# jiahansu/GPUAR

Hardware: AMD Instinct MI355X
Metric: encode+decode GB/s (higher is better)
Workload: dtype u16

## Files before the change

gpuar_amd/csrc/gpuar_kernels.hip:

```cpp
#include <hip/hip_runtime.h>
#include <mutex>
#include <stdint.h>
#include <stdio.h>
#include <stdlib.h>
#include <string.h>

#include "gpuar_hip.h"

#include "lane_codec.h"
#include "crc32.h"
#include "planes.h"

namespace gpuar {

__constant__ RecipTable g_recip = RecipTable();
struct MulTable {
    uint32_t m[kPacket + 64];
    constexpr MulTable() : m{} {
        const RecipTable r = RecipTable();
        for (uint32_t i = 0; i < kPacket + 64; ++i) m[i] = r.r[i < kPacket ? i : kPacket - 1u].mul;
    }
};
__device__ const MulTable g_mul = MulTable();
__constant__ DecodeConstTable g_decode = DecodeConstTable();
__device__ uint32_t g_status = 0;
__device__ uint32_t g_status_taken;
__device__ uint32_t g_cu_ticket[2048];
constexpr uint32_t kClockSlots = 256, kClockEvery = 64;
__device__ unsigned long long g_clock_samples[2][kClockSlots][4];
__device__ __forceinline__ void clock_sample(uint32_t which, size_t group, uint32_t lane, uint32_t end) {
    if ((group & (kClockEvery - 1u)) == 0u && group < size_t(kClockSlots) * kClockEvery && lane == 0u) {
        unsigned long long *slot = g_clock_samples[which][group / kClockEvery] + 2u * end;
        slot[0] = clock64();
        slot[1] = wall_clock64();
    }
}

__device__ __forceinline__ uint32_t lane_column(uint32_t lane) {
    return ((lane & 31u) << 1) | (lane >> 5);
}

__device__ __forceinline__ uint32_t wave_max(uint32_t v) {
#pragma unroll
    for (int off = 32; off > 0; off >>= 1) {
        const uint32_t other = __shfl_xor(v, off);
        v = other > v ? other : v;
    }
    return __builtin_amdgcn_readfirstlane(v);
}

constexpr uint32_t kPhase = 8;
constexpr int kPrioTop = 3, kPrioCoder = 0, kPrioLow = 2;

constexpr uint32_t kRingSlots = 3;
struct alignas(16) EncodeLds {
    uint8_t tree[kTreeRows * kLanes * 2];
    uint32_t sums[kRingSlots][kPhase][kLanes];
    uint32_t bytes[2][kPhase / 4][kLanes];
};
__device__ __forceinline__ uint32_t next_slot(uint32_t slot) { return slot == kRingSlots - 1u ? 0u : slot + 1u; }

__device__ __forceinline__ size_t xcd_contiguous_group(uint32_t block, uint32_t grid) {
    const uint32_t per_xcd = grid >> 3;
    return static_cast<size_t>(block & 7u) * per_xcd + (block >> 3);
}

__device__ __forceinline__ void lds_barrier() {
    asm volatile("s_waitcnt lgkmcnt(0)\n\ts_barrier" ::: "memory");
}

__device__ __forceinline__ uint4 load16_guarded(const uint8_t *p, size_t avail) {
    if (avail >= 16) return *reinterpret_cast<const uint4 *>(p);
    uint32_t w[4] = {0, 0, 0, 0};
    for (size_t b = 0; b < avail; ++b) w[b >> 2] |= static_cast<uint32_t>(p[b]) << (8u * (b & 3u));
    return make_uint4(w[0], w[1], w[2], w[3]);
}
// ... 991 lines not shown

#define GPUAR_STREAM_EVEN_TAKE  \
            "v_add_u32 %[pc], %[no], %[ne]\n\t"  \
            "v_sub_co_u32 %[raw], %[sb], %[rem], %[pc]\n\t"  \
            "v_and_b32 %[rem], 31, %[raw]\n\t"
#define GPUAR_STREAM_EVEN_WINDOW  \
            "v_perm_b32 %[pa], 0, %[ahead], %[bsw]\n\t"  \
            "v_cndmask_b32 %[w0], %[w0], %[w1], %[sb]\n\t" \
            "v_cndmask_b32 %[w1], %[w1], %[pa], %[sb]\n\t" \
            "v_alignbit_b32 v216, %[w0], %[w1], %[rem]\n\t"
#define GPUAR_STREAM_ODD_MOVE  \
            "v_lshrrev_b32 %[pb], 31, %[raw]\n\t"  \
            "v_lshl_add_u32 %[next], %[pb], 8, %[next]\n\t" \
            "v_and_or_b32 %[pc], %[next], %[kf00], %[ring]\n\t"  \
            "ds_read_b32 %[ahead], %[pc]\n\t"

#define GPUAR_OFF_TEXT(N) \
            "v_lshlrev_b64 v[216:217], %[" N "], v[216:217]\n\t"

#define GPUAR_STEP_OPERANDS_COMMON \
              [R0] "=&v"(R0), [R] "=&v"(R), [np] "=&v"(np), [am] "=&v"(am), [t0] "=&v"(t0), [t1] "=&v"(t1), [t2] "=&v"(t2), [t3] "=&v"(t3), \
              [m0] "=&s"(m0), [m1] "=&s"(m1), [ma] "=&s"(ma), [mc] "=&s"(mc), [mj] "=&s"(mj), [sx] "=&s"(sx), [sb] "=&s"(sb), [raw] "+v"(rem_raw), \
              [root] "+v"(dec.model.root), [h0] "+v"(dec.model.half0), [h1] "+v"(dec.model.half1), \
              [rng] "+v"(dec.range), [off] "+v"(offr), [kff] "+v"(kff), [oaddr] "+v"(oaddr), \
              [rem] "+v"(dec.rem), [w0] "+v"(dec.w0), [w1] "+v"(dec.w1), [ahead] "+v"(dec.ahead), [next] "+v"(next64), "+v"(window), \
              [dn] "=&v"(dn), [bw] "=&v"(bw), [cc] "=&v"(cc), [pa] "=&v"(pa), [pb] "=&v"(pb), [pc] "=&v"(pc), [ps] "=&v"(ps), \
              [wd] "=&v"(wd), [h] "=&v"(h), [e] "=&v"(e)

#define GPUAR_STEP_LOCALS \
        uint32_t R0, R, np, am, t0, t1, t2, t3, dn, bw, cc, pa, pb, pc, ps, wd, h, e; \
        unsigned long long m0, m1, ma, mc, mj, sx, sb;

#define GPUAR_STEP_EVEN_TEXT(SHADOW, OWN_ADDRESS, J, MUL, WORD) \
    GPUAR_STEP_HEAD                                 \
    SHADOW GPUAR_TOTAL_STEP GPUAR_REG_NODES GPUAR_STREAM_EVEN_TAKE \
    "s_waitcnt lgkmcnt(1)\n\t"                      \
    GPUAR_MID_WALK                                  \
    GPUAR_STREAM_EVEN_WINDOW \
    "s_waitcnt lgkmcnt(1)\n\t"                      \
    GPUAR_LOW_WALK(OWN_ADDRESS) GPUAR_LOW_INTERVAL(MUL) GPUAR_STEP_END("ne") GPUAR_FILE_SYMBOL(J, WORD) GPUAR_OFF_TEXT("ne")
#define GPUAR_STEP_ODD_TEXT(SHADOW, OWN_ADDRESS, J, MUL, WORD) \
    GPUAR_STEP_HEAD \
    SHADOW GPUAR_TOTAL_STEP GPUAR_STREAM_ODD_MOVE \
    "s_waitcnt lgkmcnt(2)\n\t"                      \
    GPUAR_MID_WALK \
    GPUAR_REG_NODES \
    "s_waitcnt lgkmcnt(1)\n\t"                      \
    GPUAR_LOW_WALK(OWN_ADDRESS) GPUAR_LOW_INTERVAL(MUL) GPUAR_STEP_END("no") GPUAR_FILE_SYMBOL(J, WORD) GPUAR_OFF_TEXT("no")
#define GPUAR_STEP_FIRST(J, MUL, WORD) GPUAR_STEP_EVEN_TEXT(GPUAR_SHADOW_PLAIN, , J, MUL, WORD)
#define GPUAR_STEP_EVEN(J, MUL, WORD) GPUAR_STEP_EVEN_TEXT(GPUAR_SHADOW_DEFERRED, , J, MUL, WORD)
#define GPUAR_STEP_ODD(J, MUL, WORD) GPUAR_STEP_ODD_TEXT(GPUAR_SHADOW_DEFERRED, , J, MUL, WORD)
#define GPUAR_STEP_LAST(J, MUL, WORD) GPUAR_STEP_ODD_TEXT(GPUAR_SHADOW_DEFERRED, GPUAR_LOW_ADDRESS_NOW, J, MUL, WORD)

constexpr uint32_t kRingPieces = 4;
constexpr uint32_t kDecodeLdsQuads = (kDecodeRecords + kRingPieces) * kLanes;

template <bool kBatch = false>
__device__ __forceinline__ void decode_wave(uint8_t *col, uint8_t *ring, const uint8_t *base, uint32_t pkt_off, uint32_t limit_off,
                                            uint8_t *out, bool live, uint32_t *status, uint32_t room = kPacket) {
    DecoderLane<9> dec;
    dec.template open<kBatch>(col, base, pkt_off, limit_off, live, room);
    const uint32_t len_max = wave_max(dec.ulen);
    uint32_t i = 0;

    const uint32_t col_lds = static_cast<uint32_t>(reinterpret_cast<uintptr_t>(col));
    const uint32_t ring_lds = static_cast<uint32_t>(reinterpret_cast<uintptr_t>(ring));
    if ((ring_lds & 0xF00u) != 0u) {
        atomicOr(status, GPUAR_STATUS_BAD_PACKET);
        return;
    }
    register uint32_t o0 asm("v204");
    register uint32_t o1 asm("v205");
    register uint32_t offr asm("v217");
    offr = dec.off | (dec.lo << 16);
    uint32_t n_even = 0, n_odd = dec.owed_bits;
    uint32_t total_v = 256u;
    uint32_t rem_raw = 0;
    register uint32_t window asm("v216");
    asm volatile("v_mov_b32 %0, 0" : "=v"(window));
    const uint32_t col_low_lds = col_lds + SubtreeModel<9>::kLowBase;
    uint32_t oaddr = col_lds + dec.model.owed.at;
    uint32_t kff = 0xFFFFu;
    const uint32_t k64k = 0x10000u, k64k1 = 0x10001u;
    const uint32_t minus_half = 0xFFFF8000u;
    uint32_t bswap_sel, ring_wrap, low_half;
    asm volatile("s_mov_b32 %0, 0xffff" : "=s"(low_half));
    asm volatile("s_mov_b32 %0, 0x00010203" : "=s"(bswap_sel));
    asm volatile("s_movk_i32 %0, 0xf00" : "=s"(ring_wrap));

    const uint32_t skew16 = static_cast<uint32_t>(reinterpret_cast<uintptr_t>(base) & 15u);
    const uint8_t *base16 = base - skew16;
    const uint32_t next16 = dec.next + skew16;
    uint32_t next64 = (next16 - 4u) << 6;
    const uint32_t last_piece = (dec.last + skew16) & ~15u;
    const uint32_t first_piece = (next16 - 4u) & ~15u;
    uint32_t fill = first_piece + 16u * kRingPieces;
    register uint32_t q0 asm("v220");
    register uint32_t q1 asm("v221");
    register uint32_t q2 asm("v222");
    register uint32_t q3 asm("v223");
    uint32_t slot_lds = ring_lds;
#pragma unroll
    for (uint32_t k = 0; k < kRingPieces; ++k) {
        const uint32_t at = first_piece + 16u * k;
        const Quad q = load128(base16 + (at < last_piece ? at : last_piece));
        uint32_t *slot = reinterpret_cast<uint32_t *>(ring + ((at & 0x30u) << 6));
        slot[0] = q.w[0], slot[64] = q.w[1], slot[128] = q.w[2], slot[192] = q.w[3];
        if (k == kRingPieces - 1u) {
            q0 = q.w[0], q1 = q.w[1], q2 = q.w[2], q3 = q.w[3];
            slot_lds = ring_lds + ((at & 0x30u) << 6);
        }
    }
#define GPUAR_RING_PHASE_TEXT(TUPLE_LO, TUPLE_HI)                                                                    \
            "v_lshrrev_b32 %[rt], 6, %[next]\n\t"                                                                    \
            "v_sub_u32 %[rt], %[fill], %[rt]\n\t"                                                                    \
            "v_cmp_gt_u32 vcc, 49, %[rt]\n\t"  \
            "s_waitcnt vmcnt(0)\n\t"                                                                                 \
            "ds_write2st64_b32 %[slot], v220, v221 offset1:1\n\t"                                                    \
            "ds_write2st64_b32 %[slot], v222, v223 offset0:2 offset1:3\n\t"                                          \
            "global_load_dwordx4 " TUPLE_LO ", %[zero], %[mulbase] offset:%[roff]\n\t"                               \
            "global_load_dwordx4 " TUPLE_HI ", %[zero], %[mulbase] offset:%[roff]+16\n\t"                            \
            "s_and_saveexec_b64 %[sx], vcc\n\t"                                                                      \
            "v_min_u32 %[rt], %[fill], %[lastp]\n\t"                                                                 \
            "global_load_dwordx4 v[220:223], %[rt], %[base]\n\t"                                                     \
            "v_and_b32 %[t2], 48, %[fill]\n\t"                                                                       \
            "v_lshl_add_u32 %[slot], %[t2], 6, %[ring]\n\t"                                                          \
            "v_add_u32 %[fill], 16, %[fill]\n\t"                                                                     \
            "s_or_b64 exec, exec, %[sx]"

    register uint32_t m00 asm("v224"); register uint32_t m01 asm("v225"); register uint32_t m02 asm("v226"); register uint32_t m03 asm("v227"); register uint32_t m04 asm("v228"); register uint32_t m05 asm("v229"); register uint32_t m06 asm("v230"); register uint32_t m07 asm("v231");
    register uint32_t m10 asm("v232"); register uint32_t m11 asm("v233"); register uint32_t m12 asm("v234"); register uint32_t m13 asm("v235"); register uint32_t m14 asm("v236"); register uint32_t m15 asm("v237"); register uint32_t m16 asm("v238"); register uint32_t m17 asm("v239");
    register uint32_t m20 asm("v240"); register uint32_t m21 asm("v241"); register uint32_t m22 asm("v242"); register uint32_t m23 asm("v243"); register uint32_t m24 asm("v244"); register uint32_t m25 asm("v245"); register uint32_t m26 asm("v246"); register uint32_t m27 asm("v247");
    register uint32_t m30 asm("v248"); register uint32_t m31 asm("v249"); register uint32_t m32 asm("v250"); register uint32_t m33 asm("v251"); register uint32_t m34 asm("v252"); register uint32_t m35 asm("v253"); register uint32_t m36 asm("v254"); register uint32_t m37 asm("v255");
    uint32_t vzero;
    asm volatile("v_mov_b32 %0, 0" : "=v"(vzero));
#define GPUAR_DECODE_RUN8(RUN, FIRST_KIND, LAST_KIND, WORD_A, WORD_B, SET_AHEAD, TUPLE_LO, TUPLE_HI)                         \
        {                                                                                                            \
            GPUAR_STEP_LOCALS                                                                                        \
            uint32_t lbw_, lcc_, ti_, path7_, rt_;                                                                   \
            unsigned long long lma_;                                                                                 \
            asm volatile(                                                                                            \
                FIRST_KIND(0, "mul0", "wa") GPUAR_STEP_ODD(1, "mul1", "wa") GPUAR_STEP_EVEN(2, "mul2", "wa") GPUAR_STEP_ODD(3, "mul3", "wa") \
                GPUAR_STEP_EVEN(0, "mul4", "wb") GPUAR_STEP_ODD(1, "mul5", "wb") GPUAR_STEP_EVEN(2, "mul6", "wb") LAST_KIND(3, "mul7", "wb") \
                 \
                GPUAR_RING_PHASE_TEXT(TUPLE_LO, TUPLE_HI)                                                            \
                : GPUAR_STEP_OPERANDS_COMMON,                                                                        \
                  [lbw] "=&v"(lbw_), [lcc] "=&v"(lcc_), [ti] "=&v"(ti_), [lma] "=&s"(lma_), [wa] "+v"(WORD_A), [wb] "+v"(WORD_B),     \
                  "+v"(o0), "+v"(o1), [c6] "+v"(path6), [c7] "=&v"(path7_), [ne] "+v"(n_even), [no] "+v"(n_odd), [totv] "+v"(total_v), \
                  [slot] "+v"(slot_lds), [fill] "+v"(fill), [rt] "=&v"(rt_), "+v"(q0), "+v"(q1), "+v"(q2), "+v"(q3),               \
                  "=v"(m##SET_AHEAD##0), "=v"(m##SET_AHEAD##1), "=v"(m##SET_AHEAD##2), "=v"(m##SET_AHEAD##3),                     \
                  "=v"(m##SET_AHEAD##4), "=v"(m##SET_AHEAD##5), "=v"(m##SET_AHEAD##6), "=v"(m##SET_AHEAD##7)                      \
                : [mul0] "v"(m##RUN##0), [mul1] "v"(m##RUN##1), [mul2] "v"(m##RUN##2), [mul3] "v"(m##RUN##3),                     \
                  [mul4] "v"(m##RUN##4), [mul5] "v"(m##RUN##5), [mul6] "v"(m##RUN##6), [mul7] "v"(m##RUN##7),                     \
                  [shift] "s"(block_shift), [col] "v"(col_lds), [collow] "v"(col_low_lds), [ring] "v"(ring_lds),                  \
                  [k64k] "v"(k64k), [k64k1] "v"(k64k1), [bsw] "s"(bswap_sel), [kf00] "s"(ring_wrap), [km32k] "s"(minus_half), [kffff] "s"(low_half), \
                  [lastp] "v"(last_piece), [base] "s"(base16), [zero] "v"(vzero), [mulbase] "s"(mul_base), [roff] "n"(32 * ((RUN) + 2))   \
                : "vcc", "scc", "memory", "v200", "v201", "v202", "v203", "v208", "v209", "v212", "v213", "v214", "v215");         \
        }
#define GPUAR_DECODE_BLOCK                                                                                           \
    {                                                                                                                \
         \
        const uint32_t block_shift = 30u - static_cast<uint32_t>(__builtin_clz(256u + i));                           \
        total_v = 256u + i;               \
        asm volatile("" : "+v"(total_v));                                                                            \
        _Pragma("unroll 1") for (uint32_t half = 0; half < 2u; ++half) {                                             \
            const uint32_t *mul_base = g_mul.m + i + 32u * half;                   \
             \
             \
            uint32_t path6;                                                                                          \
            asm volatile("" : "=v"(path6));                                                                          \
            GPUAR_DECODE_RUN8(0, GPUAR_STEP_FIRST, GPUAR_STEP_ODD, w0, w1, 2, "v[240:243]", "v[244:247]")            \
            GPUAR_DECODE_RUN8(1, GPUAR_STEP_EVEN, GPUAR_STEP_ODD, w2, w3, 3, "v[248:251]", "v[252:255]")             \
            GPUAR_DECODE_RUN8(2, GPUAR_STEP_EVEN, GPUAR_STEP_ODD, w4, w5, 0, "v[224:227]", "v[228:231]")             \
            GPUAR_DECODE_RUN8(3, GPUAR_STEP_EVEN, GPUAR_STEP_LAST, w6, w7, 1, "v[232:235]", "v[236:239]")            \
             \
             \
             \
            if (half == 0u) {                                                                                        \
                k0 = ~w0, k1 = ~w1, k2 = ~w2, k3 = ~w3, k4 = ~w4, k5 = ~w5, k6 = ~w6, k7 = ~w7;                      \
            } else {                                                                                                 \
                uint4 *dst = reinterpret_cast<uint4 *>(out + i);                                                     \
                dst[0] = make_uint4(k0, k1, k2, k3);                                                                 \
                dst[1] = make_uint4(k4, k5, k6, k7);                                                                 \
                dst[2] = make_uint4(~w0, ~w1, ~w2, ~w3);                                                             \
                dst[3] = make_uint4(~w4, ~w5, ~w6, ~w7);                                                             \
            }                                                                                                        \
        }                                                                                                            \
    }

    const uint32_t len_min = wave_max(~dec.ulen) ^ 0xFFFFFFFFu;
    asm volatile("v_mov_b32 %0, 0\n\tv_mov_b32 %1, 0" : "=v"(o0), "=v"(o1));
    uint32_t w0, w1, w2, w3, w4, w5, w6, w7;
    uint32_t k0 = 0, k1 = 0, k2 = 0, k3 = 0, k4 = 0, k5 = 0, k6 = 0, k7 = 0;
    asm volatile("v_mov_b32 %0, 0\n\tv_mov_b32 %1, 0\n\tv_mov_b32 %2, 0\n\tv_mov_b32 %3, 0\n\tv_mov_b32 %4, 0\n\tv_mov_b32 %5, 0\n\tv_mov_b32 %6, 0\n\tv_mov_b32 %7, 0"
                 : "=v"(w0), "=v"(w1), "=v"(w2), "=v"(w3), "=v"(w4), "=v"(w5), "=v"(w6), "=v"(w7));
    asm volatile("global_load_dwordx4 v[224:227], %[zero], %[mulbase]\n\t"
                 "global_load_dwordx4 v[228:231], %[zero], %[mulbase] offset:16\n\t"
                 "global_load_dwordx4 v[232:235], %[zero], %[mulbase] offset:32\n\t"
                 "global_load_dwordx4 v[236:239], %[zero], %[mulbase] offset:48\n\t"
                 "s_waitcnt vmcnt(0)"
                 : "=v"(m00), "=v"(m01), "=v"(m02), "=v"(m03), "=v"(m04), "=v"(m05), "=v"(m06), "=v"(m07),
                   "=v"(m10), "=v"(m11), "=v"(m12), "=v"(m13), "=v"(m14), "=v"(m15), "=v"(m16), "=v"(m17)
                 : [zero] "v"(vzero), [mulbase] "s"(static_cast<const uint32_t *>(g_mul.m))
                 : "memory");
    for (; i + 64u <= len_min; i += 64u) {
        GPUAR_DECODE_BLOCK
    }
    for (; i + 64u <= len_max; i += 64u) {
        if (i + 64u <= dec.ulen) GPUAR_DECODE_BLOCK
    }
#undef GPUAR_DECODE_BLOCK
#undef GPUAR_DECODE_RUN8

#undef GPUAR_RING_PHASE_TEXT
    asm volatile("s_waitcnt vmcnt(0) lgkmcnt(0)" : "+v"(dec.ahead), "+v"(q0), "+v"(q1), "+v"(q2), "+v"(q3) : : "memory");
    dec.next = (next64 >> 6) + 4u - skew16;
    dec.off = offr & 0xFFFFu;
    dec.lo = (offr >> 16) & 0x7FFFu;
    dec.owed_bits = n_even + n_odd;
    asm volatile("ds_add_u64 %[oaddr], v[204:205]\n\ts_waitcnt lgkmcnt(0)" : "+v"(o0), "+v"(o1) : [oaddr] "v"(oaddr) : "memory");
    dec.model.owed.at = oaddr - col_lds;
    {
        const Pair now = load64(col + dec.model.owed.at);
        dec.model.owed.w0 = now.w[0], dec.model.owed.w1 = now.w[1];
    }
    const uint32_t part_from = dec.ulen & ~63u;
    const uint32_t part_end = wave_max((dec.ulen & 63u) ? dec.ulen : 0u);
    const uint32_t part_begin = wave_max((dec.ulen & 63u) ? ~part_from : 0u) ^ 0xFFFFFFFFu;
    for (i = part_begin; i < part_end; ++i) {
        const DecodeConst k = g_decode.c[i];
        if (i >= part_from && i < dec.ulen) dec.step(i, k, out);
    }
    if (live) {
        dec.finish(out);
        if (dec.bad) atomicOr(status, GPUAR_STATUS_BAD_PACKET);
    }
}

__device__ __forceinline__ const uint8_t *group_slots(const uint8_t *slots, size_t n_bytes, uint32_t lane, uint32_t &limit_off) {
    const size_t group_at = static_cast<size_t>(blockIdx.x) * (kLanes * kSlot);
    const uint8_t *base = slots + group_at;
    const size_t group_left = n_bytes - group_at;
    const uint32_t slot_end = (lane + 1u) * kSlot;
    limit_off = group_left < slot_end ? static_cast<uint32_t>(group_left) : slot_end;
    return base;
}

__global__ void __launch_bounds__(kLanes)
decode_slots_kernel(const uint8_t *__restrict__ slots, uint32_t n_packets, size_t n_bytes, uint8_t *__restrict__ out, uint32_t *__restrict__ status) {
    __shared__ __attribute__((aligned(4096))) uint4 lds[kDecodeLdsQuads];
    const uint32_t lane = threadIdx.x;
    const size_t packet = static_cast<size_t>(blockIdx.x) * kLanes + lane;
    const bool live = packet < n_packets;
    uint32_t limit_off;
    const uint8_t *base = group_slots(slots, n_bytes, lane, limit_off);
    clock_sample(1u, blockIdx.x, lane, 0u);
    decode_wave(reinterpret_cast<uint8_t *>(lds) + 8u * lane, reinterpret_cast<uint8_t *>(lds + kDecodeRecords * kLanes) + 4u * lane, base, lane * kSlot, limit_off,
                out + (live ? packet : 0) * static_cast<size_t>(kPacket), live, status);
    clock_sample(1u, blockIdx.x, lane, 1u);
}

__global__ void __launch_bounds__(kLanes)
decode_stream_kernel(const uint8_t *__restrict__ stream, const uint64_t *__restrict__ offsets,
                     uint32_t n_packets, uint8_t *__restrict__ out, uint32_t *__restrict__ status) {
    __shared__ __attribute__((aligned(4096))) uint4 lds[kDecodeLdsQuads];
    const uint32_t lane = threadIdx.x;
    const size_t packet = static_cast<size_t>(blockIdx.x) * kLanes + lane;
    const bool live = packet < n_packets;
    const uint64_t first = offsets[static_cast<size_t>(blockIdx.x) * kLanes] & ~3ull;
    const uint32_t first_hi = static_cast<uint32_t>(__builtin_amdgcn_readfirstlane(static_cast<int>(static_cast<uint32_t>(first >> 32))));
    const uint32_t first_lo = static_cast<uint32_t>(__builtin_amdgcn_readfirstlane(static_cast<int>(static_cast<uint32_t>(first))));
    const uint8_t *group_stream = stream + ((static_cast<uint64_t>(first_hi) << 32) | first_lo);
    const uint64_t left = offsets[n_packets] - first;
    const uint32_t limit_off = left < 0x7FFFFFFFull ? static_cast<uint32_t>(left) : 0x7FFFFFFFu;
    const uint32_t pkt_off = live ? static_cast<uint32_t>(offsets[packet] - first) : 0u;
    clock_sample(1u, blockIdx.x, lane, 0u);
    decode_wave(reinterpret_cast<uint8_t *>(lds) + 8u * lane, reinterpret_cast<uint8_t *>(lds + kDecodeRecords * kLanes) + 4u * lane, group_stream, pkt_off, limit_off,
                out + (live ? packet : 0) * static_cast<size_t>(kPacket), live, status);
    clock_sample(1u, blockIdx.x, lane, 1u);
}

__device__ __forceinline__ bool batch_output(uint8_t *const *outs, const uint64_t *out_bytes, const uint64_t *first_packet, uint32_t n_buffers,
                                             size_t packet, bool live, uint8_t *&out, uint32_t &room, uint32_t *status) {
    out = nullptr;
    room = 0u;
    if (!live) return false;
    const BatchLane bl = batch_lane(reinterpret_cast<const uint8_t *const *>(outs), out_bytes, first_packet, n_buffers, packet);
    if (!bl.owned || bl.count == 0u) {
        atomicOr(status, GPUAR_STATUS_BAD_BATCH);
        return false;
    }
    out = const_cast<uint8_t *>(bl.ptr);
    room = bl.count;
    return true;
}

__global__ void __launch_bounds__(kLanes)
decode_slots_batch_kernel(const uint8_t *__restrict__ slots, const uint64_t *__restrict__ first_packet, uint32_t n_buffers, uint32_t n_packets,
                          uint8_t *const *__restrict__ outs, const uint64_t *__restrict__ out_bytes, uint32_t *__restrict__ status) {
    __shared__ __attribute__((aligned(4096))) uint4 lds[kDecodeLdsQuads];
    const uint32_t lane = threadIdx.x;
    const size_t packet = static_cast<size_t>(blockIdx.x) * kLanes + lane;
    uint32_t limit_off;
    const uint8_t *base = group_slots(slots, static_cast<size_t>(n_packets) * kSlot, lane, limit_off);
    uint8_t *out;
    uint32_t room;
    const bool live = batch_output(outs, out_bytes, first_packet, n_buffers, packet, packet < n_packets, out, room, status);
    decode_wave<true>(reinterpret_cast<uint8_t *>(lds) + 8u * lane, reinterpret_cast<uint8_t *>(lds + kDecodeRecords * kLanes) + 4u * lane, base, lane * kSlot, limit_off,
                      out, live, status, room);
}

__global__ void __launch_bounds__(kLanes)
decode_stream_batch_kernel(const uint8_t *__restrict__ stream, const uint64_t *__restrict__ offsets, const uint64_t *__restrict__ first_packet,
                           uint32_t n_buffers, uint32_t n_packets, uint8_t *const *__restrict__ outs, const uint64_t *__restrict__ out_bytes,
                           uint32_t *__restrict__ status) {
    __shared__ __attribute__((aligned(4096))) uint4 lds[kDecodeLdsQuads];
    const uint32_t lane = threadIdx.x;
    const size_t packet = static_cast<size_t>(blockIdx.x) * kLanes + lane;
    const bool in_range = packet < n_packets;
    const uint64_t first = offsets[static_cast<size_t>(blockIdx.x) * kLanes] & ~3ull;
    const uint32_t first_hi = static_cast<uint32_t>(__builtin_amdgcn_readfirstlane(static_cast<int>(static_cast<uint32_t>(first >> 32))));
    const uint32_t first_lo = static_cast<uint32_t>(__builtin_amdgcn_readfirstlane(static_cast<int>(static_cast<uint32_t>(first))));
    const uint8_t *group_stream = stream + ((static_cast<uint64_t>(first_hi) << 32) | first_lo);
    const uint64_t left = offsets[n_packets] - first;
    const uint32_t limit_off = left < 0x7FFFFFFFull ? static_cast<uint32_t>(left) : 0x7FFFFFFFu;
    const uint32_t pkt_off = in_range ? static_cast<uint32_t>(offsets[packet] - first) : 0u;
    uint8_t *out;
    uint32_t room;
    const bool live = batch_output(outs, out_bytes, first_packet, n_buffers, packet, in_range, out, room, status);
    decode_wave<true>(reinterpret_cast<uint8_t *>(lds) + 8u * lane, reinterpret_cast<uint8_t *>(lds + kDecodeRecords * kLanes) + 4u * lane, group_stream, pkt_off, limit_off,
                      out, live, status, room);
// ... 468 lines not shown
inline bool aligned16(const void *p) { return (reinterpret_cast<uintptr_t>(p) & 15u) == 0; }

int check_launch() {
    const hipError_t e = hipGetLastError();
    return e == hipSuccess ? GPUAR_OK : static_cast<int>(e);
}

uint32_t *status_word(uint32_t *d_status) {
    if (d_status) return d_status;
    void *p = nullptr;
    if (hipGetSymbolAddress(&p, HIP_SYMBOL(gpuar::g_status)) != hipSuccess) return nullptr;
    return static_cast<uint32_t *>(p);
}

}

extern "C" {

size_t gpuar_hip_packet_count(size_t n_bytes) { return (n_bytes + GPUAR_PACKET_BYTES - 1) / GPUAR_PACKET_BYTES; }

int gpuar_hip_encode_mode(const uint8_t *d_in, size_t n_bytes, uint8_t *d_slots, uint32_t *d_status, void *stream, int mode) {
    if (mode != GPUAR_MODE_AUTO && mode != GPUAR_MODE_THROUGHPUT && mode != GPUAR_MODE_LATENCY) return GPUAR_ERR_ARGUMENT;
    if (n_bytes == 0) return GPUAR_OK;
    if (!d_in || !d_slots) return GPUAR_ERR_ARGUMENT;
    if (!aligned16(d_in) || !aligned16(d_slots) || (reinterpret_cast<uintptr_t>(d_status) & 3u)) return GPUAR_ERR_ALIGNMENT;
    uint32_t *status = status_word(d_status);
    if (!status) return GPUAR_ERR_NO_DEVICE;
    const size_t n_packets = gpuar_hip_packet_count(n_bytes);
    if (n_packets > 0xFFFFFFFFull) return GPUAR_ERR_ARGUMENT;
    const uint32_t groups = static_cast<uint32_t>((n_packets + gpuar::kLanes - 1) / gpuar::kLanes);
    const bool latency = mode == GPUAR_MODE_LATENCY || (mode == GPUAR_MODE_AUTO && groups <= gpuar::kSmallGroups);
    if (latency) {
        gpuar::encode_small_kernel<<<groups, gpuar::kSmallWaves * gpuar::kLanes, 0, static_cast<hipStream_t>(stream)>>>(
            d_in, n_bytes, d_slots, static_cast<uint32_t>(n_packets), status);
        return check_launch();
    }
    const uint32_t blocks = (groups + 7u) & ~7u;
    gpuar::encode_kernel<<<blocks, 4 * gpuar::kLanes, 0, static_cast<hipStream_t>(stream)>>>(
        d_in, n_bytes, d_slots, static_cast<uint32_t>(n_packets), status);
    return check_launch();
}

int gpuar_hip_encode(const uint8_t *d_in, size_t n_bytes, uint8_t *d_slots, uint32_t *d_status, void *stream) {
    return gpuar_hip_encode_mode(d_in, n_bytes, d_slots, d_status, stream, GPUAR_MODE_AUTO);
}

static int launch_decode_slots(const uint8_t *d_slots, size_t n_packets, size_t n_bytes, uint8_t *d_out, uint32_t *d_status, void *stream) {
    if (n_packets == 0) return GPUAR_OK;
    if (!d_slots || !d_out || n_packets > 0xFFFFFFFFull) return GPUAR_ERR_ARGUMENT;
    if (!aligned16(d_slots) || !aligned16(d_out) || (reinterpret_cast<uintptr_t>(d_status) & 3u)) return GPUAR_ERR_ALIGNMENT;
    uint32_t *status = status_word(d_status);
    if (!status) return GPUAR_ERR_NO_DEVICE;
    const uint32_t blocks = static_cast<uint32_t>((n_packets + gpuar::kLanes - 1) / gpuar::kLanes);
    gpuar::decode_slots_kernel<<<blocks, gpuar::kLanes, 0, static_cast<hipStream_t>(stream)>>>(
        d_slots, static_cast<uint32_t>(n_packets), n_bytes, d_out, status);
    return check_launch();
}

int gpuar_hip_decode(const uint8_t *d_slots, size_t n_packets, uint8_t *d_out, uint32_t *d_status, void *stream) {
    return launch_decode_slots(d_slots, n_packets, n_packets * static_cast<size_t>(GPUAR_SLOT_BYTES), d_out, d_status, stream);
}

int gpuar_hip_compact(const uint8_t *d_slots, size_t n_packets, uint8_t *d_stream, uint64_t *d_offsets, void *stream) {
    if (!d_offsets) return GPUAR_ERR_ARGUMENT;
    hipStream_t s = static_cast<hipStream_t>(stream);
    if (n_packets == 0) {
        const hipError_t e = hipMemsetAsync(d_offsets, 0, sizeof(uint64_t), s);
        return e == hipSuccess ? GPUAR_OK : static_cast<int>(e);
    }
    if (!d_slots || !d_stream) return GPUAR_ERR_ARGUMENT;
    if (!aligned16(d_slots) || (reinterpret_cast<uintptr_t>(d_offsets) & 7u) || (reinterpret_cast<uintptr_t>(d_stream) & 7u))
        return GPUAR_ERR_ALIGNMENT;
    if (n_packets * static_cast<size_t>(gpuar::kGatherThreads) > 0xFFFFFFFFull) return GPUAR_ERR_ARGUMENT;
    const size_t tiles = (n_packets + gpuar::kScanTile - 1) / gpuar::kScanTile;
    const uint32_t np = static_cast<uint32_t>(n_packets);
    uint64_t *tile_prefix = tiles > 1 ? reinterpret_cast<uint64_t *>(d_stream) : nullptr;
    if (tile_prefix) {
        gpuar::scan_tile_sums_kernel<<<static_cast<uint32_t>(tiles), gpuar::kScanThreads, 0, s>>>(d_slots, np, tile_prefix);
        gpuar::scan_tile_prefix_kernel<<<1, gpuar::kScanThreads, 0, s>>>(static_cast<uint32_t>(tiles), tile_prefix);
    }
    gpuar::scan_offsets_kernel<<<static_cast<uint32_t>(tiles), gpuar::kScanThreads, 0, s>>>(d_slots, np, d_offsets, tile_prefix);
    gpuar::gather_kernel<<<np, gpuar::kGatherThreads, 0, s>>>(d_slots, d_offsets, np, d_stream);
    return check_launch();
}

int gpuar_hip_decode_stream(const uint8_t *d_stream, const uint64_t *d_offsets, size_t n_packets,
                            uint8_t *d_out, uint32_t *d_status, void *stream) {
    if (n_packets == 0) return GPUAR_OK;
    if (!d_stream || !d_offsets || !d_out || n_packets > 0xFFFFFFFFull) return GPUAR_ERR_ARGUMENT;
    if (!aligned16(d_out) || (reinterpret_cast<uintptr_t>(d_stream) & 3u) || (reinterpret_cast<uintptr_t>(d_status) & 3u)) return GPUAR_ERR_ALIGNMENT;
    uint32_t *status = status_word(d_status);
    if (!status) return GPUAR_ERR_NO_DEVICE;
    const uint32_t blocks = static_cast<uint32_t>((n_packets + gpuar::kLanes - 1) / gpuar::kLanes);
    gpuar::decode_stream_kernel<<<blocks, gpuar::kLanes, 0, static_cast<hipStream_t>(stream)>>>(
        d_stream, d_offsets, static_cast<uint32_t>(n_packets), d_out, status);
    return check_launch();
}

size_t gpuar_hip_batch_packet_count(const uint64_t *bytes, size_t n_buffers, uint64_t *first_packet) {
    if (n_buffers && !bytes) return 0;
    size_t total = 0;
    for (size_t b = 0; b < n_buffers; ++b) {
        if (first_packet) first_packet[b] = total;
        total += gpuar_hip_packet_count(bytes[b]);
    }
    if (first_packet) first_packet[n_buffers] = total;
    return total;
}

static int batch_arguments(const void *d_ptrs, const uint64_t *d_bytes, const uint64_t *d_first_packet, size_t n_buffers,
                           size_t n_packets, const void *d_packets, uintptr_t packets_align, uint32_t *d_status, uint32_t **status_out) {
    if (!d_ptrs || !d_bytes || !d_first_packet || !d_packets) return GPUAR_ERR_ARGUMENT;
    if (n_packets > 0xFFFFFFFFull || n_buffers > 0xFFFFFFFFull) return GPUAR_ERR_ARGUMENT;
    if ((reinterpret_cast<uintptr_t>(d_ptrs) & 7u) || (reinterpret_cast<uintptr_t>(d_bytes) & 7u) ||
        (reinterpret_cast<uintptr_t>(d_first_packet) & 7u) || (reinterpret_cast<uintptr_t>(d_status) & 3u) ||
        (reinterpret_cast<uintptr_t>(d_packets) & (packets_align - 1u)))
        return GPUAR_ERR_ALIGNMENT;
    *status_out = status_word(d_status);
    return *status_out ? GPUAR_OK : GPUAR_ERR_NO_DEVICE;
}

int gpuar_hip_encode_batch(const uint8_t *const *d_in_ptrs, const uint64_t *d_in_bytes, const uint64_t *d_first_packet,
                           size_t n_buffers, size_t n_packets, uint8_t *d_slots, uint32_t *d_status, void *stream, int mode) {
    if (mode != GPUAR_MODE_AUTO && mode != GPUAR_MODE_THROUGHPUT && mode != GPUAR_MODE_LATENCY) return GPUAR_ERR_ARGUMENT;
    if (n_packets == 0) return GPUAR_OK;
    uint32_t *status = nullptr;
    const int e = batch_arguments(d_in_ptrs, d_in_bytes, d_first_packet, n_buffers, n_packets, d_slots, 16u, d_status, &status);
    if (e != GPUAR_OK) return e;
    const uint32_t groups = static_cast<uint32_t>((n_packets + gpuar::kLanes - 1) / gpuar::kLanes);
    hipStream_t s = static_cast<hipStream_t>(stream);
    const bool latency = mode == GPUAR_MODE_LATENCY || (mode == GPUAR_MODE_AUTO && groups <= gpuar::kSmallGroups);
    if (latency) {
        gpuar::encode_small_batch_kernel<<<groups, gpuar::kSmallWaves * gpuar::kLanes, 0, s>>>(
            d_in_ptrs, d_in_bytes, d_first_packet, static_cast<uint32_t>(n_buffers), static_cast<uint32_t>(n_packets), d_slots, status);
        return check_launch();
    }
    const uint32_t blocks = (groups + 7u) & ~7u;
    gpuar::encode_batch_kernel<<<blocks, 4 * gpuar::kLanes, 0, s>>>(
        d_in_ptrs, d_in_bytes, d_first_packet, static_cast<uint32_t>(n_buffers), static_cast<uint32_t>(n_packets), d_slots, status);
    return check_launch();
}

int gpuar_hip_decode_batch(const uint8_t *d_slots, const uint64_t *d_first_packet, size_t n_buffers, size_t n_packets,
                           uint8_t *const *d_out_ptrs, const uint64_t *d_out_bytes, uint32_t *d_status, void *stream) {
    if (n_packets == 0) return GPUAR_OK;
    uint32_t *status = nullptr;
    const int e = batch_arguments(d_out_ptrs, d_out_bytes, d_first_packet, n_buffers, n_packets, d_slots, 16u, d_status, &status);
    if (e != GPUAR_OK) return e;
// ... 326 lines not shown
```

Baseline: 202.7.

## Add wide decode path with interleaved step table precomputing per-symbol totals

Adds a step table that interleaves the reciprocal multiplier with a precomputed total (256+i) for each position. A new wide decode loop loads 16 table registers per 8-symbol run instead of 8, so each step uses a single v_mad_u32_u16 with the precomputed total instead of tracking a running total. Both the slot and stream decode entry points switch to new wide kernels whenever at least two groups are launched. In exchange the loop holds 64 more pinned VGPRs and issues twice as many table loads per run, which adds register pressure and memory traffic.

```diff
diff --git a/gpuar_amd/csrc/gpuar_kernels.hip b/gpuar_amd/csrc/gpuar_kernels.hip
--- a/gpuar_amd/csrc/gpuar_kernels.hip
+++ b/gpuar_amd/csrc/gpuar_kernels.hip
@@ -22,6 +22,14 @@
     }
 };
 __device__ const MulTable g_mul = MulTable();
+struct StepTable {
+    uint32_t v[2 * (kPacket + 64)];
+    constexpr StepTable() : v{} {
+        const RecipTable r = RecipTable();
+        for (uint32_t i = 0; i < kPacket + 64; ++i) v[2 * i] = r.r[i < kPacket ? i : kPacket - 1u].mul, v[2 * i + 1] = 256u + i;
+    }
+};
+__device__ const StepTable g_step = StepTable();
 __constant__ DecodeConstTable g_decode = DecodeConstTable();
 __device__ uint32_t g_status = 0;
 __device__ uint32_t g_status_taken;
@@ -1119,10 +1127,45 @@
 #define GPUAR_STEP_ODD(J, MUL, WORD) GPUAR_STEP_ODD_TEXT(GPUAR_SHADOW_DEFERRED, , J, MUL, WORD)
 #define GPUAR_STEP_LAST(J, MUL, WORD) GPUAR_STEP_ODD_TEXT(GPUAR_SHADOW_DEFERRED, GPUAR_LOW_ADDRESS_NOW, J, MUL, WORD)
 
+#define GPUAR_STEP2_HEAD(TOT, TM1)  \
+            "v_mad_u32_u16 %[R0], %[off], %[" TOT "], %[" TM1 "]\n\t"  \
+            "v_mul_u32_u24 %[t0], %[root], %[rng]\n\t" \
+            "v_sub_co_u32 %[t1], %[m0], %[R0], %[t0]\n\t"  \
+            "v_min_u32 %[R], %[R0], %[t1]\n\t" \
+            "v_cndmask_b32 %[t2], %[h1], %[h0], %[m0]\n\t"  \
+            "v_mul_u32_u24 %[t0], %[t2], %[rng]\n\t" \
+            "v_sub_co_u32 %[t1], %[m1], %[R], %[t0]\n\t" \
+            "v_cndmask_b32 %[np], 0, 2, %[m0]\n\t" \
+            "v_addc_co_u32 %[np], vcc, %[np], 0, %[m1]\n\t"  \
+            "v_lshl_add_u32 %[am], %[np], 10, %[col]\n\t" \
+            "ds_read2_b64 v[200:203], %[am] offset1:64\n\t"  \
+            "v_min_u32 %[R], %[R], %[t1]\n\t"
+
+#define GPUAR_STEP2_EVEN_TEXT(SHADOW, OWN_ADDRESS, J, MUL, WORD, TOT, TM1) \
+    GPUAR_STEP2_HEAD(TOT, TM1) \
+    SHADOW GPUAR_REG_NODES GPUAR_STREAM_EVEN_TAKE \
+    "s_waitcnt lgkmcnt(1)\n\t" \
+    GPUAR_MID_WALK \
+    GPUAR_STREAM_EVEN_WINDOW \
+    "s_waitcnt lgkmcnt(1)\n\t" \
+    GPUAR_LOW_WALK(OWN_ADDRESS) GPUAR_LOW_INTERVAL(MUL) GPUAR_STEP_END("ne") GPUAR_FILE_SYMBOL(J, WORD) GPUAR_OFF_TEXT("ne")
+#define GPUAR_STEP2_ODD_TEXT(SHADOW, OWN_ADDRESS, J, MUL, WORD, TOT, TM1) \
+    GPUAR_STEP2_HEAD(TOT, TM1) \
+    SHADOW GPUAR_STREAM_ODD_MOVE \
+    "s_waitcnt lgkmcnt(2)\n\t" \
+    GPUAR_MID_WALK \
+    GPUAR_REG_NODES \
+    "s_waitcnt lgkmcnt(1)\n\t" \
+    GPUAR_LOW_WALK(OWN_ADDRESS) GPUAR_LOW_INTERVAL(MUL) GPUAR_STEP_END("no") GPUAR_FILE_SYMBOL(J, WORD) GPUAR_OFF_TEXT("no")
+#define GPUAR_STEP2_FIRST(J, MUL, WORD, TOT, TM1) GPUAR_STEP2_EVEN_TEXT(GPUAR_SHADOW_PLAIN, , J, MUL, WORD, TOT, TM1)
+#define GPUAR_STEP2_EVEN(J, MUL, WORD, TOT, TM1) GPUAR_STEP2_EVEN_TEXT(GPUAR_SHADOW_DEFERRED, , J, MUL, WORD, TOT, TM1)
+#define GPUAR_STEP2_ODD(J, MUL, WORD, TOT, TM1) GPUAR_STEP2_ODD_TEXT(GPUAR_SHADOW_DEFERRED, , J, MUL, WORD, TOT, TM1)
+#define GPUAR_STEP2_LAST(J, MUL, WORD, TOT, TM1) GPUAR_STEP2_ODD_TEXT(GPUAR_SHADOW_DEFERRED, GPUAR_LOW_ADDRESS_NOW, J, MUL, WORD, TOT, TM1)
+
 constexpr uint32_t kRingPieces = 4;
 constexpr uint32_t kDecodeLdsQuads = (kDecodeRecords + kRingPieces) * kLanes;
 
-template <bool kBatch = false>
+template <bool kBatch = false, bool kWide = false>
 __device__ __forceinline__ void decode_wave(uint8_t *col, uint8_t *ring, const uint8_t *base, uint32_t pkt_off, uint32_t limit_off,
                                             uint8_t *out, bool live, uint32_t *status, uint32_t room = kPacket) {
     DecoderLane<9> dec;
@@ -1199,6 +1242,10 @@
     register uint32_t m10 asm("v232"); register uint32_t m11 asm("v233"); register uint32_t m12 asm("v234"); register uint32_t m13 asm("v235"); register uint32_t m14 asm("v236"); register uint32_t m15 asm("v237"); register uint32_t m16 asm("v238"); register uint32_t m17 asm("v239");
     register uint32_t m20 asm("v240"); register uint32_t m21 asm("v241"); register uint32_t m22 asm("v242"); register uint32_t m23 asm("v243"); register uint32_t m24 asm("v244"); register uint32_t m25 asm("v245"); register uint32_t m26 asm("v246"); register uint32_t m27 asm("v247");
     register uint32_t m30 asm("v248"); register uint32_t m31 asm("v249"); register uint32_t m32 asm("v250"); register uint32_t m33 asm("v251"); register uint32_t m34 asm("v252"); register uint32_t m35 asm("v253"); register uint32_t m36 asm("v254"); register uint32_t m37 asm("v255");
+    [[maybe_unused]] register uint32_t x0_0 asm("v128"); [[maybe_unused]] register uint32_t x0_1 asm("v129"); [[maybe_unused]] register uint32_t x0_2 asm("v130"); [[maybe_unused]] register uint32_t x0_3 asm("v131"); [[maybe_unused]] register uint32_t x0_4 asm("v132"); [[maybe_unused]] register uint32_t x0_5 asm("v133"); [[maybe_unused]] register uint32_t x0_6 asm("v134"); [[maybe_unused]] register uint32_t x0_7 asm("v135"); [[maybe_unused]] register uint32_t x0_8 asm("v136"); [[maybe_unused]] register uint32_t x0_9 asm("v137"); [[maybe_unused]] register uint32_t x0_10 asm("v138"); [[maybe_unused]] register uint32_t x0_11 asm("v139"); [[maybe_unused]] register uint32_t x0_12 asm("v140"); [[maybe_unused]] register uint32_t x0_13 asm("v141"); [[maybe_unused]] register uint32_t x0_14 asm("v142"); [[maybe_unused]] register uint32_t x0_15 asm("v143");
+    [[maybe_unused]] register uint32_t x1_0 asm("v144"); [[maybe_unused]] register uint32_t x1_1 asm("v145"); [[maybe_unused]] register uint32_t x1_2 asm("v146"); [[maybe_unused]] register uint32_t x1_3 asm("v147"); [[maybe_unused]] register uint32_t x1_4 asm("v148"); [[maybe_unused]] register uint32_t x1_5 asm("v149"); [[maybe_unused]] register uint32_t x1_6 asm("v150"); [[maybe_unused]] register uint32_t x1_7 asm("v151"); [[maybe_unused]] register uint32_t x1_8 asm("v152"); [[maybe_unused]] register uint32_t x1_9 asm("v153"); [[maybe_unused]] register uint32_t x1_10 asm("v154"); [[maybe_unused]] register uint32_t x1_11 asm("v155"); [[maybe_unused]] register uint32_t x1_12 asm("v156"); [[maybe_unused]] register uint32_t x1_13 asm("v157"); [[maybe_unused]] register uint32_t x1_14 asm("v158"); [[maybe_unused]] register uint32_t x1_15 asm("v159");
+    [[maybe_unused]] register uint32_t x2_0 asm("v160"); [[maybe_unused]] register uint32_t x2_1 asm("v161"); [[maybe_unused]] register uint32_t x2_2 asm("v162"); [[maybe_unused]] register uint32_t x2_3 asm("v163"); [[maybe_unused]] register uint32_t x2_4 asm("v164"); [[maybe_unused]] register uint32_t x2_5 asm("v165"); [[maybe_unused]] register uint32_t x2_6 asm("v166"); [[maybe_unused]] register uint32_t x2_7 asm("v167"); [[maybe_unused]] register uint32_t x2_8 asm("v168"); [[maybe_unused]] register uint32_t x2_9 asm("v169"); [[maybe_unused]] register uint32_t x2_10 asm("v170"); [[maybe_unused]] register uint32_t x2_11 asm("v171"); [[maybe_unused]] register uint32_t x2_12 asm("v172"); [[maybe_unused]] register uint32_t x2_13 asm("v173"); [[maybe_unused]] register uint32_t x2_14 asm("v174"); [[maybe_unused]] register uint32_t x2_15 asm("v175");
+    [[maybe_unused]] register uint32_t x3_0 asm("v176"); [[maybe_unused]] register uint32_t x3_1 asm("v177"); [[maybe_unused]] register uint32_t x3_2 asm("v178"); [[maybe_unused]] register uint32_t x3_3 asm("v179"); [[maybe_unused]] register uint32_t x3_4 asm("v180"); [[maybe_unused]] register uint32_t x3_5 asm("v181"); [[maybe_unused]] register uint32_t x3_6 asm("v182"); [[maybe_unused]] register uint32_t x3_7 asm("v183"); [[maybe_unused]] register uint32_t x3_8 asm("v184"); [[maybe_unused]] register uint32_t x3_9 asm("v185"); [[maybe_unused]] register uint32_t x3_10 asm("v186"); [[maybe_unused]] register uint32_t x3_11 asm("v187"); [[maybe_unused]] register uint32_t x3_12 asm("v188"); [[maybe_unused]] register uint32_t x3_13 asm("v189"); [[maybe_unused]] register uint32_t x3_14 asm("v190"); [[maybe_unused]] register uint32_t x3_15 asm("v191");
     uint32_t vzero;
     asm volatile("v_mov_b32 %0, 0" : "=v"(vzero));
 #define GPUAR_DECODE_RUN8(RUN, FIRST_KIND, LAST_KIND, WORD_A, WORD_B, SET_AHEAD, TUPLE_LO, TUPLE_HI)                         \
@@ -1215,13 +1262,61 @@
                   [lbw] "=&v"(lbw_), [lcc] "=&v"(lcc_), [ti] "=&v"(ti_), [lma] "=&s"(lma_), [wa] "+v"(WORD_A), [wb] "+v"(WORD_B),     \
                   "+v"(o0), "+v"(o1), [c6] "+v"(path6), [c7] "=&v"(path7_), [ne] "+v"(n_even), [no] "+v"(n_odd), [totv] "+v"(total_v), \
                   [slot] "+v"(slot_lds), [fill] "+v"(fill), [rt] "=&v"(rt_), "+v"(q0), "+v"(q1), "+v"(q2), "+v"(q3),               \
-                  "=v"(m##SET_AHEAD##0), "=v"(m##SET_AHEAD##1), "=v"(m##SET_AHEAD##2), "=v"(m##SET_AHEAD##3),                     \
-                  "=v"(m##SET_AHEAD##4), "=v"(m##SET_AHEAD##5), "=v"(m##SET_AHEAD##6), "=v"(m##SET_AHEAD##7)                      \
+                  "=&v"(m##SET_AHEAD##0), "=&v"(m##SET_AHEAD##1), "=&v"(m##SET_AHEAD##2), "=&v"(m##SET_AHEAD##3),                     \
+                  "=&v"(m##SET_AHEAD##4), "=&v"(m##SET_AHEAD##5), "=&v"(m##SET_AHEAD##6), "=&v"(m##SET_AHEAD##7)                      \
                 : [mul0] "v"(m##RUN##0), [mul1] "v"(m##RUN##1), [mul2] "v"(m##RUN##2), [mul3] "v"(m##RUN##3),                     \
                   [mul4] "v"(m##RUN##4), [mul5] "v"(m##RUN##5), [mul6] "v"(m##RUN##6), [mul7] "v"(m##RUN##7),                     \
                   [shift] "s"(block_shift), [col] "v"(col_lds), [collow] "v"(col_low_lds), [ring] "v"(ring_lds),                  \
                   [k64k] "v"(k64k), [k64k1] "v"(k64k1), [bsw] "s"(bswap_sel), [kf00] "s"(ring_wrap), [km32k] "s"(minus_half), [kffff] "s"(low_half), \
                   [lastp] "v"(last_piece), [base] "s"(base16), [zero] "v"(vzero), [mulbase] "s"(mul_base), [roff] "n"(32 * ((RUN) + 2))   \
+                : "vcc", "scc", "memory", "v200", "v201", "v202", "v203", "v208", "v209", "v212", "v213", "v214", "v215");         \
+        }
+#define GPUAR_RING_PHASE_TEXT_WIDE(T0, T1, T2, T3)                                                                   \
+            "v_lshrrev_b32 %[rt], 6, %[next]\n\t"                                                                    \
+            "v_sub_u32 %[rt], %[fill], %[rt]\n\t"                                                                    \
+            "v_cmp_gt_u32 vcc, 49, %[rt]\n\t"                                                                        \
+            "s_waitcnt vmcnt(0)\n\t"                                                                                 \
+            "ds_write2st64_b32 %[slot], v220, v221 offset1:1\n\t"                                                    \
+            "ds_write2st64_b32 %[slot], v222, v223 offset0:2 offset1:3\n\t"                                          \
+            "global_load_dwordx4 " T0 ", %[zero], %[mulbase] offset:%[roff]\n\t"                                     \
+            "global_load_dwordx4 " T1 ", %[zero], %[mulbase] offset:%[roff]+16\n\t"                                  \
+            "global_load_dwordx4 " T2 ", %[zero], %[mulbase] offset:%[roff]+32\n\t"                                  \
+            "global_load_dwordx4 " T3 ", %[zero], %[mulbase] offset:%[roff]+48\n\t"                                  \
+            "s_and_saveexec_b64 %[sx], vcc\n\t"                                                                      \
+            "v_min_u32 %[rt], %[fill], %[lastp]\n\t"                                                                 \
+            "global_load_dwordx4 v[220:223], %[rt], %[base]\n\t"                                                     \
+            "v_and_b32 %[t2], 48, %[fill]\n\t"                                                                       \
+            "v_lshl_add_u32 %[slot], %[t2], 6, %[ring]\n\t"                                                          \
+            "v_add_u32 %[fill], 16, %[fill]\n\t"                                                                     \
+            "s_or_b64 exec, exec, %[sx]"
+#define GPUAR_DECODE_RUN8_WIDE(RUN, PREV, FIRST_KIND, LAST_KIND, WORD_A, WORD_B, SET_AHEAD, T0, T1, T2, T3)           \
+        {                                                                                                            \
+            GPUAR_STEP_LOCALS                                                                                        \
+            uint32_t lbw_, lcc_, ti_, path7_, rt_;                                                                   \
+            unsigned long long lma_;                                                                                 \
+            asm volatile(                                                                                            \
+                FIRST_KIND(0, "mul0", "wa", "tot0", "totp") GPUAR_STEP2_ODD(1, "mul1", "wa", "tot1", "tot0")         \
+                GPUAR_STEP2_EVEN(2, "mul2", "wa", "tot2", "tot1") GPUAR_STEP2_ODD(3, "mul3", "wa", "tot3", "tot2")   \
+                GPUAR_STEP2_EVEN(0, "mul4", "wb", "tot4", "tot3") GPUAR_STEP2_ODD(1, "mul5", "wb", "tot5", "tot4")   \
+                GPUAR_STEP2_EVEN(2, "mul6", "wb", "tot6", "tot5") LAST_KIND(3, "mul7", "wb", "tot7", "tot6")         \
+                 \
+                GPUAR_RING_PHASE_TEXT_WIDE(T0, T1, T2, T3)                                                           \
+                : GPUAR_STEP_OPERANDS_COMMON,                                                                        \
+                  [lbw] "=&v"(lbw_), [lcc] "=&v"(lcc_), [ti] "=&v"(ti_), [lma] "=&s"(lma_), [wa] "+v"(WORD_A), [wb] "+v"(WORD_B),     \
+                  "+v"(o0), "+v"(o1), [c6] "+v"(path6), [c7] "=&v"(path7_), [ne] "+v"(n_even), [no] "+v"(n_odd),                       \
+                  [slot] "+v"(slot_lds), [fill] "+v"(fill), [rt] "=&v"(rt_), "+v"(q0), "+v"(q1), "+v"(q2), "+v"(q3),               \
+                  "=&v"(x##SET_AHEAD##_0), "=&v"(x##SET_AHEAD##_1), "=&v"(x##SET_AHEAD##_2), "=&v"(x##SET_AHEAD##_3),               \
+                  "=&v"(x##SET_AHEAD##_4), "=&v"(x##SET_AHEAD##_5), "=&v"(x##SET_AHEAD##_6), "=&v"(x##SET_AHEAD##_7),               \
+                  "=&v"(x##SET_AHEAD##_8), "=&v"(x##SET_AHEAD##_9), "=&v"(x##SET_AHEAD##_10), "=&v"(x##SET_AHEAD##_11),             \
+                  "=&v"(x##SET_AHEAD##_12), "=&v"(x##SET_AHEAD##_13), "=&v"(x##SET_AHEAD##_14), "=&v"(x##SET_AHEAD##_15)            \
+                : [mul0] "v"(x##RUN##_0), [mul1] "v"(x##RUN##_2), [mul2] "v"(x##RUN##_4), [mul3] "v"(x##RUN##_6),                   \
+                  [mul4] "v"(x##RUN##_8), [mul5] "v"(x##RUN##_10), [mul6] "v"(x##RUN##_12), [mul7] "v"(x##RUN##_14),                \
+                  [tot0] "v"(x##RUN##_1), [tot1] "v"(x##RUN##_3), [tot2] "v"(x##RUN##_5), [tot3] "v"(x##RUN##_7),                   \
+                  [tot4] "v"(x##RUN##_9), [tot5] "v"(x##RUN##_11), [tot6] "v"(x##RUN##_13), [tot7] "v"(x##RUN##_15),                \
+                  [totp] "v"(x##PREV##_15),                                                                                         \
+                  [shift] "s"(block_shift), [col] "v"(col_lds), [collow] "v"(col_low_lds), [ring] "v"(ring_lds),                  \
+                  [k64k] "v"(k64k), [k64k1] "v"(k64k1), [bsw] "s"(bswap_sel), [kf00] "s"(ring_wrap), [km32k] "s"(minus_half), [kffff] "s"(low_half), \
+                  [lastp] "v"(last_piece), [base] "s"(base16), [zero] "v"(vzero), [mulbase] "s"(step_base), [roff] "n"(64 * ((RUN) + 2))  \
                 : "vcc", "scc", "memory", "v200", "v201", "v202", "v203", "v208", "v209", "v212", "v213", "v214", "v215");         \
         }
 #define GPUAR_DECODE_BLOCK                                                                                           \
@@ -1255,12 +1350,60 @@
         }                                                                                                            \
     }
 
+#define GPUAR_DECODE_BLOCK_WIDE                                                                                      \
+    {                                                                                                                \
+        const uint32_t block_shift = 30u - static_cast<uint32_t>(__builtin_clz(256u + i));                           \
+        _Pragma("unroll 1") for (uint32_t half = 0; half < 2u; ++half) {                                             \
+            const uint32_t *step_base = g_step.v + 2u * (i + 32u * half);           \
+            uint32_t path6;                                                                                          \
+            asm volatile("" : "=v"(path6));                                                                          \
+            GPUAR_DECODE_RUN8_WIDE(0, 3, GPUAR_STEP2_FIRST, GPUAR_STEP2_ODD, w0, w1, 2, "v[160:163]", "v[164:167]", "v[168:171]", "v[172:175]") \
+            GPUAR_DECODE_RUN8_WIDE(1, 0, GPUAR_STEP2_EVEN, GPUAR_STEP2_ODD, w2, w3, 3, "v[176:179]", "v[180:183]", "v[184:187]", "v[188:191]")  \
+            GPUAR_DECODE_RUN8_WIDE(2, 1, GPUAR_STEP2_EVEN, GPUAR_STEP2_ODD, w4, w5, 0, "v[128:131]", "v[132:135]", "v[136:139]", "v[140:143]")  \
+            GPUAR_DECODE_RUN8_WIDE(3, 2, GPUAR_STEP2_EVEN, GPUAR_STEP2_LAST, w6, w7, 1, "v[144:147]", "v[148:151]", "v[152:155]", "v[156:159]") \
+            if (half == 0u) {                                                                                        \
+                k0 = ~w0, k1 = ~w1, k2 = ~w2, k3 = ~w3, k4 = ~w4, k5 = ~w5, k6 = ~w6, k7 = ~w7;                      \
+            } else {                                                                                                 \
+                uint4 *dst = reinterpret_cast<uint4 *>(out + i);                                                     \
+                dst[0] = make_uint4(k0, k1, k2, k3);                                                                 \
+                dst[1] = make_uint4(k4, k5, k6, k7);                                                                 \
+                dst[2] = make_uint4(~w0, ~w1, ~w2, ~w3);                                                             \
+                dst[3] = make_uint4(~w4, ~w5, ~w6, ~w7);                                                             \
+            }                                                                                                        \
+        }                                                                                                            \
+    }
+
     const uint32_t len_min = wave_max(~dec.ulen) ^ 0xFFFFFFFFu;
     asm volatile("v_mov_b32 %0, 0\n\tv_mov_b32 %1, 0" : "=v"(o0), "=v"(o1));
     uint32_t w0, w1, w2, w3, w4, w5, w6, w7;
     uint32_t k0 = 0, k1 = 0, k2 = 0, k3 = 0, k4 = 0, k5 = 0, k6 = 0, k7 = 0;
     asm volatile("v_mov_b32 %0, 0\n\tv_mov_b32 %1, 0\n\tv_mov_b32 %2, 0\n\tv_mov_b32 %3, 0\n\tv_mov_b32 %4, 0\n\tv_mov_b32 %5, 0\n\tv_mov_b32 %6, 0\n\tv_mov_b32 %7, 0"
                  : "=v"(w0), "=v"(w1), "=v"(w2), "=v"(w3), "=v"(w4), "=v"(w5), "=v"(w6), "=v"(w7));
+    if constexpr (kWide) {
+        asm volatile("global_load_dwordx4 v[128:131], %[zero], %[stepbase]\n\t"
+                     "global_load_dwordx4 v[132:135], %[zero], %[stepbase] offset:16\n\t"
+                     "global_load_dwordx4 v[136:139], %[zero], %[stepbase] offset:32\n\t"
+                     "global_load_dwordx4 v[140:143], %[zero], %[stepbase] offset:48\n\t"
+                     "global_load_dwordx4 v[144:147], %[zero], %[stepbase] offset:64\n\t"
+                     "global_load_dwordx4 v[148:151], %[zero], %[stepbase] offset:80\n\t"
+                     "global_load_dwordx4 v[152:155], %[zero], %[stepbase] offset:96\n\t"
+                     "global_load_dwordx4 v[156:159], %[zero], %[stepbase] offset:112\n\t"
+                     "v_mov_b32 %[before], 0xff\n\t"
+                     "s_waitcnt vmcnt(0)"
+                     : "=v"(x0_0), "=v"(x0_1), "=v"(x0_2), "=v"(x0_3), "=v"(x0_4), "=v"(x0_5), "=v"(x0_6), "=v"(x0_7),
+                       "=v"(x0_8), "=v"(x0_9), "=v"(x0_10), "=v"(x0_11), "=v"(x0_12), "=v"(x0_13), "=v"(x0_14), "=v"(x0_15),
+                       "=v"(x1_0), "=v"(x1_1), "=v"(x1_2), "=v"(x1_3), "=v"(x1_4), "=v"(x1_5), "=v"(x1_6), "=v"(x1_7),
+                       "=v"(x1_8), "=v"(x1_9), "=v"(x1_10), "=v"(x1_11), "=v"(x1_12), "=v"(x1_13), "=v"(x1_14), "=v"(x1_15),
+                       [before] "=v"(x3_15)
+                     : [zero] "v"(vzero), [stepbase] "s"(static_cast<const uint32_t *>(g_step.v))
+                     : "memory");
+        for (; i + 64u <= len_min; i += 64u) {
+            GPUAR_DECODE_BLOCK_WIDE
+        }
+        for (; i + 64u <= len_max; i += 64u) {
+            if (i + 64u <= dec.ulen) GPUAR_DECODE_BLOCK_WIDE
+        }
+    } else {
     asm volatile("global_load_dwordx4 v[224:227], %[zero], %[mulbase]\n\t"
                  "global_load_dwordx4 v[228:231], %[zero], %[mulbase] offset:16\n\t"
                  "global_load_dwordx4 v[232:235], %[zero], %[mulbase] offset:32\n\t"
@@ -1276,8 +1419,12 @@
     for (; i + 64u <= len_max; i += 64u) {
         if (i + 64u <= dec.ulen) GPUAR_DECODE_BLOCK
     }
+    }
 #undef GPUAR_DECODE_BLOCK
+#undef GPUAR_DECODE_BLOCK_WIDE
 #undef GPUAR_DECODE_RUN8
+#undef GPUAR_DECODE_RUN8_WIDE
+#undef GPUAR_RING_PHASE_TEXT_WIDE
 
 #undef GPUAR_RING_PHASE_TEXT
     asm volatile("s_waitcnt vmcnt(0) lgkmcnt(0)" : "+v"(dec.ahead), "+v"(q0), "+v"(q1), "+v"(q2), "+v"(q3) : : "memory");
@@ -1344,6 +1491,42 @@
     clock_sample(1u, blockIdx.x, lane, 0u);
     decode_wave(reinterpret_cast<uint8_t *>(lds) + 8u * lane, reinterpret_cast<uint8_t *>(lds + kDecodeRecords * kLanes) + 4u * lane, group_stream, pkt_off, limit_off,
                 out + (live ? packet : 0) * static_cast<size_t>(kPacket), live, status);
+    clock_sample(1u, blockIdx.x, lane, 1u);
+}
+
+constexpr uint32_t kWideGroups = 2;
+
+__global__ void __launch_bounds__(kLanes)
+decode_slots_wide_kernel(const uint8_t *__restrict__ slots, uint32_t n_packets, size_t n_bytes, uint8_t *__restrict__ out, uint32_t *__restrict__ status) {
+    __shared__ __attribute__((aligned(4096))) uint4 lds[kDecodeLdsQuads];
+    const uint32_t lane = threadIdx.x;
+    const size_t packet = static_cast<size_t>(blockIdx.x) * kLanes + lane;
+    const bool live = packet < n_packets;
+    uint32_t limit_off;
+    const uint8_t *base = group_slots(slots, n_bytes, lane, limit_off);
+    clock_sample(1u, blockIdx.x, lane, 0u);
+    decode_wave<false, true>(reinterpret_cast<uint8_t *>(lds) + 8u * lane, reinterpret_cast<uint8_t *>(lds + kDecodeRecords * kLanes) + 4u * lane, base, lane * kSlot,
+                             limit_off, out + (live ? packet : 0) * static_cast<size_t>(kPacket), live, status);
+    clock_sample(1u, blockIdx.x, lane, 1u);
+}
+
+__global__ void __launch_bounds__(kLanes)
+decode_stream_wide_kernel(const uint8_t *__restrict__ stream, const uint64_t *__restrict__ offsets,
+                          uint32_t n_packets, uint8_t *__restrict__ out, uint32_t *__restrict__ status) {
+    __shared__ __attribute__((aligned(4096))) uint4 lds[kDecodeLdsQuads];
+    const uint32_t lane = threadIdx.x;
+    const size_t packet = static_cast<size_t>(blockIdx.x) * kLanes + lane;
+    const bool live = packet < n_packets;
+    const uint64_t first = offsets[static_cast<size_t>(blockIdx.x) * kLanes] & ~3ull;
+    const uint32_t first_hi = static_cast<uint32_t>(__builtin_amdgcn_readfirstlane(static_cast<int>(static_cast<uint32_t>(first >> 32))));
+    const uint32_t first_lo = static_cast<uint32_t>(__builtin_amdgcn_readfirstlane(static_cast<int>(static_cast<uint32_t>(first))));
+    const uint8_t *group_stream = stream + ((static_cast<uint64_t>(first_hi) << 32) | first_lo);
+    const uint64_t left = offsets[n_packets] - first;
+    const uint32_t limit_off = left < 0x7FFFFFFFull ? static_cast<uint32_t>(left) : 0x7FFFFFFFu;
+    const uint32_t pkt_off = live ? static_cast<uint32_t>(offsets[packet] - first) : 0u;
+    clock_sample(1u, blockIdx.x, lane, 0u);
+    decode_wave<false, true>(reinterpret_cast<uint8_t *>(lds) + 8u * lane, reinterpret_cast<uint8_t *>(lds + kDecodeRecords * kLanes) + 4u * lane, group_stream, pkt_off,
+                             limit_off, out + (live ? packet : 0) * static_cast<size_t>(kPacket), live, status);
     clock_sample(1u, blockIdx.x, lane, 1u);
 }
 
@@ -1918,8 +2101,12 @@
     uint32_t *status = status_word(d_status);
     if (!status) return GPUAR_ERR_NO_DEVICE;
     const uint32_t blocks = static_cast<uint32_t>((n_packets + gpuar::kLanes - 1) / gpuar::kLanes);
-    gpuar::decode_slots_kernel<<<blocks, gpuar::kLanes, 0, static_cast<hipStream_t>(stream)>>>(
-        d_slots, static_cast<uint32_t>(n_packets), n_bytes, d_out, status);
+    if (blocks >= gpuar::kWideGroups)
+        gpuar::decode_slots_wide_kernel<<<blocks, gpuar::kLanes, 0, static_cast<hipStream_t>(stream)>>>(
+            d_slots, static_cast<uint32_t>(n_packets), n_bytes, d_out, status);
+    else
+        gpuar::decode_slots_kernel<<<blocks, gpuar::kLanes, 0, static_cast<hipStream_t>(stream)>>>(
+            d_slots, static_cast<uint32_t>(n_packets), n_bytes, d_out, status);
     return check_launch();
 }
 
@@ -1958,8 +2145,12 @@
     uint32_t *status = status_word(d_status);
     if (!status) return GPUAR_ERR_NO_DEVICE;
     const uint32_t blocks = static_cast<uint32_t>((n_packets + gpuar::kLanes - 1) / gpuar::kLanes);
-    gpuar::decode_stream_kernel<<<blocks, gpuar::kLanes, 0, static_cast<hipStream_t>(stream)>>>(
-        d_stream, d_offsets, static_cast<uint32_t>(n_packets), d_out, status);
+    if (blocks >= gpuar::kWideGroups)
+        gpuar::decode_stream_wide_kernel<<<blocks, gpuar::kLanes, 0, static_cast<hipStream_t>(stream)>>>(
+            d_stream, d_offsets, static_cast<uint32_t>(n_packets), d_out, status);
+    else
+        gpuar::decode_stream_kernel<<<blocks, gpuar::kLanes, 0, static_cast<hipStream_t>(stream)>>>(
+            d_stream, d_offsets, static_cast<uint32_t>(n_packets), d_out, status);
     return check_launch();
 }
 
```

Measured after the change: 203.9 (median of 6 runs). No clear change (+0.6%).
